# mspaintenjoyer/DepthEstimation

Hardware: AMD Instinct MI355X
Metric: disparity Mpix/s at 1080p d_max=128; 1/2/4/8-GPU scaling + %HBM roofline (higher is better)
Workload: dtype u8

## Files before the change

### depthestimation_amd/csrc/dsx_bm.hip

```cpp
#include "dsx_internal.h"
#include "dsx_partition.h"
#include "dsx_subpix.h"

constexpr int kWpe = 3;
constexpr int kWpeSsd = 4;

#ifndef DSX_ROWSTEP_PAIRTAIL
#define DSX_ROWSTEP_PAIRTAIL 0
#endif
#ifndef DSX_ROWSTEP_DIVQ
#define DSX_ROWSTEP_DIVQ 1
#endif
#ifndef DSX_ROWSTEP_OVERLAP
#define DSX_ROWSTEP_OVERLAP 1
#endif
#ifndef DSX_ROWSTEP_AHEAD
#define DSX_ROWSTEP_AHEAD 1
#endif
#ifndef DSX_ROWSTEP_SREF
#define DSX_ROWSTEP_SREF 0
#endif
#ifndef DSX_ROWSTEP_SARGS
#define DSX_ROWSTEP_SARGS DSX_ROWSTEP_SREF
#endif
constexpr bool kRowstepSref = DSX_ROWSTEP_SREF;
constexpr bool kRowstepSargs = DSX_ROWSTEP_SARGS;
constexpr bool kRowstepOverlap = DSX_ROWSTEP_OVERLAP;
constexpr bool kRowstepAhead = DSX_ROWSTEP_AHEAD;
constexpr bool kRowstepPairtail = DSX_ROWSTEP_PAIRTAIL;
constexpr bool kRowstepDivq = DSX_ROWSTEP_DIVQ;
#ifndef DSX_ROWSTEP_ATID
#define DSX_ROWSTEP_ATID 1
#endif
#ifndef DSX_ROWSTEP_KEY2
#define DSX_ROWSTEP_KEY2 1
#endif
#ifndef DSX_ROWSTEP_MERGE
#define DSX_ROWSTEP_MERGE 1
#endif
constexpr bool kRowstepMerge = DSX_ROWSTEP_MERGE;
constexpr bool kRowstepAtid = DSX_ROWSTEP_ATID;
constexpr bool kRowstepKey2 = DSX_ROWSTEP_KEY2;
#ifndef DSX_SEGSTART_AHEAD
#define DSX_SEGSTART_AHEAD 1
#endif
#ifndef DSX_SEGSTART_BATCH
#define DSX_SEGSTART_BATCH 1
#endif
#ifndef DSX_SEGSTART_SPART
#define DSX_SEGSTART_SPART 0
#endif
constexpr bool kSegstartAhead = DSX_SEGSTART_AHEAD;
constexpr bool kSegstartBatch = DSX_SEGSTART_BATCH;
constexpr bool kSegstartSpart = DSX_SEGSTART_SPART;

#include <algorithm>
#include <cstdio>
#include <cstdlib>
#include <cstring>
#include <mutex>
#include <type_traits>
#include <utility>
#include <vector>

namespace dsx {

typedef unsigned short u16x2 __attribute__((ext_vector_type(2)));
typedef uint32_t u32x2 __attribute__((ext_vector_type(2)));
__device__ __forceinline__ u32x2 lds_read_b64(const uint8_t *p) {
    return *(const volatile __attribute__((address_space(3))) u32x2 *)p;
}

__device__ __forceinline__ u16x2 as2(uint32_t v) { return __builtin_bit_cast(u16x2, v); }
__device__ __forceinline__ uint32_t as1(u16x2 v) { return __builtin_bit_cast(uint32_t, v); }
__device__ __forceinline__ int clampi2(int v, int lo, int hi) { return v < lo ? lo : (v > hi ? hi : v); }
__device__ __forceinline__ uint32_t umin2(uint32_t a, uint32_t b) { return a < b ? a : b; }
__device__ __forceinline__ u16x2 add_sub2(u16x2 a, u16x2 p, u16x2 q) { return as2(as1(a) + as1(p) - as1(q)); }
__device__ __forceinline__ int mad_i24(int a, int b, int c) {
    int r;
    asm("v_mad_i32_i24 %0, %1, %2, %3" : "=v"(r) : "v"(a), "v"(b), "v"(c));
    return r;
}
__device__ __forceinline__ uint32_t sad_hi_u8(uint32_t a, uint32_t b, uint32_t c) {
    return __builtin_amdgcn_sad_hi_u8(a, b, c);
}
__device__ __forceinline__ uint32_t min_shr1(uint32_t src, uint32_t key) {
    asm("s_nop 1\n\tv_min_u32_dpp %0, %1, %0 wave_shr:1 row_mask:0xf bank_mask:0xf" : "+v"(key) : "v"(src));
    return key;
}
#pragma clang diagnostic push
#pragma clang diagnostic ignored "-Winline-asm"
template <int OFF0, int STRIDE>
__device__ __forceinline__ void lds_store8_addtid(uint32_t m0base, const uint32_t (&v)[8]) {
    static_assert(OFF0 >= 0 && OFF0 + 7 * STRIDE < 65536, "16-bit offset field");
    asm volatile("s_mov_b32 m0, %8\n\ts_nop 0\n\t"
                 "ds_write_addtid_b32 %0 offset:%9\n\t"
                 "ds_write_addtid_b32 %1 offset:%10\n\t"
                 "ds_write_addtid_b32 %2 offset:%11\n\t"
                 "ds_write_addtid_b32 %3 offset:%12\n\t"
                 "ds_write_addtid_b32 %4 offset:%13\n\t"
                 "ds_write_addtid_b32 %5 offset:%14\n\t"
                 "ds_write_addtid_b32 %6 offset:%15\n\t"
                 "ds_write_addtid_b32 %7 offset:%16"
                 :
// ... 100 lines not shown
#endif
) {
    using G = Geo<R, SSD, NW>;
    constexpr int TX = G::TX, NC = G::NC, Dp = G::Dp, NT = G::NT, TPP = G::TPP, DSL = G::DSL, CB = G::CB,
                  PITCH = G::PITCH, NJ = G::NJ, SLOT = G::SLOT, NB = G::NB, NJ4 = (NJ + 3) / 4;
    constexpr int side = SIDE;
    const Bm2Args a = kargs_row<SIDE == 3>(a_in);
    constexpr bool FSS = SSD && !ABS && R <= 5 && (SIDE == 0 || SIDE == 3 || SIDE == 4);
    constexpr bool SGK = SIDE == 4;
    constexpr uint32_t OFF = FSS ? 0x4B000000u : 0u;
    constexpr int CW = (!FSS && (SSD || SIDE == 3)) ? 4 : 8, NCH = (NC + CW - 1) / CW;
    typedef typename std::conditional<FSS, float, typename std::conditional<SSD, uint32_t, u16x2>::type>::type acc_t;
    uint8_t *tile = smem + 4 * SLOT;

    constexpr bool LANE_RB = SSD && !ABS && NW >= 4;
    int ln = 0;
    if constexpr (LANE_RB)
        asm volatile("v_mbcnt_lo_u32_b32 %0, -1, 0\n\tv_mbcnt_hi_u32_b32 %0, -1, %0" : "=v"(ln));
    else
        ln = (int)threadIdx.x & 63;
    const int tid = LANE_RB ? (wvu << 6) + ln : (int)threadIdx.x;
    const int wv = LANE_RB ? wvu : tid >> 6;
    const int H = a.H, W = a.W, m = a.m, D = a.D;
    const int64_t stride = a.stride;
    const int d0 = SSD ? (wv * 64 + ln) : (wv * 128 + 2 * ln);
    const uint32_t padv = a.padv;
    const int PB = side == 1 ? (x0 - R + m) : (x0 - R - m + NC - 1);
    const int sgn = side == 1 ? 1 : -1;

    constexpr int NC4 = (NC + 3) / 4;
    constexpr bool RL2 = !SSD;
    uint32_t ofs_r = (uint32_t)(x0 - R + 4 * min(tid, NC4 - 1));
    uint32_t ofs_s = side == 1 ? (uint32_t)(PB + 4 * min(tid, NJ4 - 1)) : (uint32_t)(PB - 4 * min(tid, NJ4 - 1) - 3);
    constexpr bool MRG = kRowstepMerge && RL2 && FAST && SIDE != 3 && SIDE != 2 && !(SIDE == 4 && R >= 7);
    static_assert(!MRG || NJ4 + NC4 <= NT, "merged staging: a lane per staged dword");
    const bool m_s = tid < NJ4;
    const int m_r = min(tid - NJ4, NC4 - 1);
    const uint8_t *m_base = m_s ? a.src + fin + ofs_s : a.ref + fin + (uint32_t)(x0 - R + 4 * m_r);
    const bool m_dn = m_s && side != 1;
    const uint32_t m_sel0 = m_dn ? 0x0C0C0C03u : 0x0C0C0C00u, m_sel1 = m_dn ? 0x0C0C0C02u : 0x0C0C0C01u,
                   m_sel2 = m_dn ? 0x0C0C0C01u : 0x0C0C0C02u, m_sel3 = m_dn ? 0x0C0C0C00u : 0x0C0C0C03u;
    const uint32_t m_lane = m_s ? (uint32_t)(16 * tid) : (uint32_t)(G::SROW + 16 * m_r);
    auto ldm = [&](int r, uint32_t &w) __attribute__((always_inline)) {
        const int yy = clampi2(r, 0, H - 1);
        long ro = (long)yy * stride;
        asm("" : "+s"(ro));
        w = *reinterpret_cast<const uint32_t *>(m_base + ro);
    };
    auto stm = [&](uint8_t *sp, uint32_t w) __attribute__((always_inline)) {
        if (tid < NJ4 + NC4)
            *reinterpret_cast<uint4 *>(sp) = make_uint4(__builtin_amdgcn_perm(0u, w, m_sel0), __builtin_amdgcn_perm(0u, w, m_sel1),
                                                        __builtin_amdgcn_perm(0u, w, m_sel2), __builtin_amdgcn_perm(0u, w, m_sel3));
    };
    auto ld = [&](int r, uint32_t &w0, uint32_t &w1, uint32_t &w2, uint32_t &w3, uint32_t &rf) __attribute__((always_inline)) {
        const int yy = clampi2(r, 0, H - 1);
        const uint8_t *srow_ = a.src + fin + (long)yy * stride;
        const uint8_t *rrow_ = a.ref + fin + (long)yy * stride;
        if constexpr (RL2) {
            asm("" : "+s"(srow_));
            asm("" : "+s"(rrow_));
        }
        typedef typename std::conditional<RL2, gu8, const uint8_t>::type row8;
        typedef typename std::conditional<RL2, gu32, const uint32_t>::type row32;
        typedef typename std::conditional<RL2, uint32_t, int>::type rix;
        row8 *srow = (row8 *)srow_, *rrow = (row8 *)rrow_;
        const int tr = min(tid, NC4 - 1);
        if constexpr (FAST) {
            if constexpr (RL2) {
                rf = *reinterpret_cast<row32 *>(rrow + ofs_r);
            } else {
                rf = *reinterpret_cast<row32 *>(rrow + x0 - R + 4 * tr);
            }
        } else {
            uint32_t v = 0;
#pragma unroll
            for (int q = 0; q < 4; ++q) v |= (uint32_t)rrow[(rix)clampi2(x0 - R + 4 * tr + q, 0, W - 1)] << (8 * q);
            rf = v;
        }
        if constexpr (FAST) {
            const int tj = min(tid, NJ4 - 1);
            row8 *p;
            if constexpr (RL2) {
                p = srow + ofs_s;
            } else {
                p = side == 1 ? srow + PB + 4 * tj : (SIDE == 3 && NW == 1) ? srow + (PB - 4 * tj - 3) : srow + PB - 4 * tj - 3;
            }
            w0 = *reinterpret_cast<row32 *>(p);
            if constexpr (RL2) w1 = w2 = w3 = 0;
        } else {
            uint32_t v[4];
            int t4 = 4 * tid;
            if constexpr (!SSD && NW == 1 && SIDE == 3)
                asm volatile("" : "+v"(t4));
#pragma unroll
            for (int q = 0; q < 4; ++q) {
                const int j = min(t4 + q, NJ - 1);
                const int pp = PB + sgn * j;
                uint32_t t = srow[(rix)clampi2(pp, 0, W - 1)];
                if constexpr (FSS) t = __float_as_uint((float)t);
                v[q] = t;
            }
            w0 = v[0];
            w1 = v[1];
            w2 = v[2];
            w3 = v[3];
        }
// ... 140 lines not shown
                } else {
                    w[r] = 0;
                    e[r] = 0;
                    rf[r] = 0;
                }
            }
        };
        auto itrg = [&](int g, const uint32_t(&w)[4], const uint32_t(&e)[4], const uint32_t(&rf)[4]) __attribute__((always_inline)) {
            uint32_t P[5];
#pragma unroll
            for (int q = 0; q < 4; ++q) {
                const uint32_t b = 3 - q;
                const uint32_t lo = __builtin_amdgcn_perm(w[1], w[0], 0x0C0C0000u | ((4u + b) << 8) | b);
                const uint32_t hi = __builtin_amdgcn_perm(w[3], w[2], 0x0C0C0000u | ((4u + b) << 8) | b);
                P[q] = __builtin_amdgcn_perm(hi, lo, 0x05040100u);
            }
            {
                const uint32_t lo = __builtin_amdgcn_perm(e[1], e[0], 0x0C0C0400u);
                const uint32_t hi = __builtin_amdgcn_perm(e[3], e[2], 0x0C0C0400u);
                P[4] = __builtin_amdgcn_perm(hi, lo, 0x05040100u);
            }
            if (tid < NJ4) {
                uint4 *tp = reinterpret_cast<uint4 *>(smem + g * TPG + 32 * tid);
                tp[0] = make_uint4(P[0], P[1], P[1], P[2]);
                tp[1] = make_uint4(P[2], P[3], P[3], P[4]);
            }
            if (tid < NC4) {
                uint32_t Rv[4];
#pragma unroll
                for (int k = 0; k < 4; ++k) {
                    const uint32_t lo = __builtin_amdgcn_perm(rf[1], rf[0], 0x0C0C0000u | ((4u + k) << 8) | (uint32_t)k);
                    const uint32_t hi = __builtin_amdgcn_perm(rf[3], rf[2], 0x0C0C0000u | ((4u + k) << 8) | (uint32_t)k);
                    Rv[k] = __builtin_amdgcn_perm(hi, lo, 0x05040100u);
                }
                *reinterpret_cast<uint4 *>(smem + NGR * TPG + g * RG + 16 * tid) = make_uint4(Rv[0], Rv[1], Rv[2], Rv[3]);
            }
        };
        if constexpr (IBT) {
            uint32_t w[NGR][4], e[NGR][4], rf[NGR][4];
#pragma unroll
            for (int g = 0; g < NGR; ++g) ildg(g, w[g], e[g], rf[g]);
            __builtin_amdgcn_sched_barrier(0);
#pragma unroll
            for (int g = 0; g < NGR; ++g) itrg(g, w[g], e[g], rf[g]);
        } else {
#pragma unroll 1
            for (int g = 0; g < NGR; ++g) {
                uint32_t w[4], e[4], rf[4];
                ildg(g, w, e, rf);
                itrg(g, w, e, rf);
            }
        }
        block_sync<NW>();
        const uint8_t *tb = smem + d0 * 8;
        {
        uint32_t ae[NC], ao[NC];
#pragma unroll
        for (int c = 0; c < NC; ++c) ae[c] = ao[c] = 0;
        constexpr bool IAH = kSegstartAhead && R <= 5;
        if constexpr (IAH) {
#pragma unroll 1
            for (int g = 0; g < NGR; ++g) {
                uint32_t rv[2][4], p0[2][4], p1[2][4];
                auto ird = [&](auto qc) __attribute__((always_inline)) {
                    constexpr int q = decltype(qc)::value, c0 = 4 * q, t = q & 1;
                    const uint4 rr = *reinterpret_cast<const uint4 *>(smem + NGR * TPG + g * RG + 4 * c0);
                    rv[t][0] = rr.x; rv[t][1] = rr.y; rv[t][2] = rr.z; rv[t][3] = rr.w;
#pragma unroll
                    for (int c = 0; c < 4; ++c) {
                        if (c0 + c < NC) {
                            if constexpr (ABS) {
                                p0[t][c] = *reinterpret_cast<const uint32_t *>(tb + g * TPG + (NC - 1 - c0 - c) * 8);
                            } else {
                                const uint2 pr = *reinterpret_cast<const uint2 *>(tb + g * TPG + (NC - 1 - c0 - c) * 8);
                                p0[t][c] = pr.x;
                                p1[t][c] = pr.y;
                            }
                        }
                    }
                };
                auto isad = [&](auto qc) __attribute__((always_inline)) {
                    constexpr int q = decltype(qc)::value, c0 = 4 * q, t = q & 1;
#pragma unroll
                    for (int c = 0; c < 4; ++c) {
                        if (c0 + c < NC) {
                            ae[c0 + c] = __builtin_amdgcn_sad_u8(rv[t][c], p0[t][c], ae[c0 + c]);
                            if constexpr (!ABS) ao[c0 + c] = __builtin_amdgcn_sad_u8(rv[t][c], p1[t][c], ao[c0 + c]);
                        }
                    }
                };
                auto ichunk = [&](auto qc) __attribute__((always_inline)) {
                    constexpr int q = decltype(qc)::value;
                    if constexpr (q < NC4) {
                        __builtin_amdgcn_sched_barrier(0);
                        if constexpr (q + 1 < NC4) ird(std::integral_constant<int, q + 1>{});
                        __builtin_amdgcn_sched_barrier(0);
                        isad(qc);
                    }
                };
                ird(std::integral_constant<int, 0>{});
                ichunk(std::integral_constant<int, 0>{}); ichunk(std::integral_constant<int, 1>{});
                ichunk(std::integral_constant<int, 2>{}); ichunk(std::integral_constant<int, 3>{});
                ichunk(std::integral_constant<int, 4>{}); ichunk(std::integral_constant<int, 5>{});
                ichunk(std::integral_constant<int, 6>{}); ichunk(std::integral_constant<int, 7>{});
                ichunk(std::integral_constant<int, 8>{}); ichunk(std::integral_constant<int, 9>{});
                ichunk(std::integral_constant<int, 10>{}); ichunk(std::integral_constant<int, 11>{});
// ... 47 lines not shown
        }
    }
    block_sync<NW>();
#pragma unroll 1
    for (int i = 0; i <= 2 * R; ++i) {
        uint32_t nx = 0;
#pragma unroll
        for (int q = 0; q < NCH; ++q) {
            const int c0 = CW * q;
            uint32_t sw[CW + 1], rw[CW];
            float rf8[8];
            s_chunk(i, c0, sw, nx);
            if constexpr (FSS) ref_chunkf(i, c0, rf8);
            else ref_chunk(i, c0, rw);
#pragma unroll
            for (int c = 0; c < CW; ++c) {
                if (c0 + c < NC) {
                    if constexpr (FSS) {
                        const float t = rf8[c] - __uint_as_float(sw[c]);
                        cs[c0 + c] = __builtin_fmaf(t, t, cs[c0 + c]);
                    } else if constexpr (ABS) {
                        cs[c0 + c] = __builtin_amdgcn_sad_u16(rw[c], sw[c], cs[c0 + c]);
                    } else if constexpr (SSD) {
                        const int t = (int)rw[c] - (int)sw[c];
                        cs[c0 + c] += (uint32_t)__mul24(t, t);
                    } else {
                        cs[c0 + c] = as2(sad_hi_u8(rw[c], pair_e1(sw, c), __builtin_amdgcn_sad_u8(rw[c], pair_e0(sw, c), as1(cs[c0 + c]))));
                    }
                }
            }
            if constexpr (SSD) __builtin_amdgcn_sched_barrier(0);
        }
    }
    }
    block_sync<NW>();

    for (int q = tid; q < TX * (Dp - D); q += NT) {
        const int k = q / (Dp - D), d = D + (q - k * (Dp - D));
        if constexpr (SSD) *reinterpret_cast<uint32_t *>(tile + k * PITCH + d * 4) = padv + OFF;
        else *reinterpret_cast<uint16_t *>(tile + k * PITCH + d * 2) = (uint16_t)padv;
    }
    block_sync<NW>();

    const bool edge = side == 1 && (x0 + m < 0 || x0 + TX - 1 + m + Dp - 1 > W - 1);
    const bool dodd = !SSD && (D & 1);
    const bool lane_writes = d0 < D;

    uint32_t stg = (MRG ? m_lane : (uint32_t)(16 * tid)) + (uint32_t)((2 - (yb & 1) * 2) * SLOT);
    constexpr bool PTAIL = kRowstepPairtail && !SSD && SIDE == 0 && NW == 1;
    constexpr bool DIVQ = kRowstepDivq && !SSD && SIDE == 0;
    uint32_t kp0 = 0, kp1 = 0;
    constexpr bool CUQ = !SSD && SIDE == 0 && NW == 1 && R < 6 && kRowstepKey2 && !PTAIL;
    constexpr bool OVL = kRowstepOverlap && CUQ, AHD = kRowstepAhead && CUQ;
    constexpr int CQ = 4, NQ = (NC + CQ - 1) / CQ;
    constexpr bool SREF = kRowstepSref && CUQ && FAST && OVL && R < 5;
    constexpr bool SRA = kRowstepSargs && CUQ && OVL && R < 5;
    static_assert(!SREF || NQ == NC4, "one reference dword per column chunk");
    uint32_t qn[NC4 + 1] = {}, qo[NC4 + 1] = {}, shn = 0, sho = 0;
    auto sld = [&](int r, uint32_t(&q)[NC4 + 1], uint32_t &sh) __attribute__((always_inline)) {
        const int yy = clampi2(r, 0, H - 1);
        const uintptr_t p = (uintptr_t)(a.ref + fin + (long)yy * stride + (x0 - R));
        typedef const __attribute__((address_space(4))) uint8_t cu8;
        cu8 *b = (cu8 *)(p & ~(uintptr_t)3);
#pragma unroll
        for (int i = 0; i < NC4; ++i) q[i] = *(cu32 *)(b + 4 * i);
        q[NC4] = *(cu32 *)(b + ((((uint32_t)p + 4u * NC4 - 1u) & ~3u) - ((uint32_t)p & ~3u)));
        sh = ((uint32_t)p & 3u) * 8u;
    };
    auto sbyte = [](uint32_t w, int c) __attribute__((always_inline)) -> uint32_t {
        return c == 3 ? w >> 24 : (w >> (8 * c)) & 0xFFu;
    };
    constexpr int RPS = NQ >= 10 ? 1 : 2, NRS = 8 / RPS;
    static_assert(NQ >= NRS + 2, "a column chunk per stage up to the element keys");
    const int ek = tid / TPP, eh = tid % TPP, ex = x0 + ek;
    const uint8_t *epx = tile + ek * PITCH + eh * DSL * CB;
    uint4 etv[2] = {};
    uint32_t ekmin = 0, ecb = 0, egblk = 0, ecm = 0, ecp = 0;
    int eb = 0, ef = 0, eden = 1;
    bool esp = false;
    auto emin8 = [](uint4 v) __attribute__((always_inline)) -> uint32_t {
        const u16x2 mm = __builtin_elementwise_min(__builtin_elementwise_min(as2(v.x), as2(v.y)),
                                                   __builtin_elementwise_min(as2(v.z), as2(v.w)));
        return umin2(mm.x, mm.y);
    };
    auto estage = [&](auto sc, int ey, auto rl, const Bm2Args &er) __attribute__((always_inline)) {
        constexpr int s = decltype(sc)::value;
        constexpr bool RL = decltype(rl)::value;
        auto pick = [&]() __attribute__((always_inline)) -> const Bm2Args & {
            if constexpr (RL) return er;
            else return a;
        };
        const Bm2Args &ea = pick();
        static_assert(!OVL || (NB == 8 && TPP == 2), "overlapped epilogue: 64 disparities per lane, two lanes per pixel");
        constexpr int GB = Dp / 8 <= 16 ? 4 : (Dp / 8 <= 32 ? 5 : 6);
        if constexpr (s <= NRS) {
            if constexpr (s == 0) ekmin = 0xFFFFFFFFu;
#pragma unroll
            for (int j = 0; j < (s > 0 ? RPS : 0); ++j) ekmin = umin2(ekmin, (emin8(etv[j]) << GB) | (uint32_t)(RPS * (s - 1) + j));
            if constexpr (s < NRS) {
#pragma unroll
                for (int j = 0; j < RPS; ++j) etv[j] = *reinterpret_cast<const uint4 *>(epx + 16 * (RPS * s + j));
            } else {
                const uint32_t kmin = gmin<TPP>(ekmin | (uint32_t)(eh * 8));
                ecb = kmin >> GB;
                egblk = kmin & ((1u << GB) - 1u);
                etv[0] = *reinterpret_cast<const uint4 *>(epx + 16 * (egblk & 7u));
            }
        } else if constexpr (s == NRS + 1) {
            const uint32_t w4[4] = {etv[0].x, etv[0].y, etv[0].z, etv[0].w};
            uint32_t k8 = 0xFFFFFFFFu;
#pragma unroll
            for (int q = 0; q < 4; ++q) {
                k8 = umin2(k8, (w4[q] << 16) | (uint32_t)(2 * q));
                k8 = umin2(k8, (w4[q] & 0xFFFF0000u) | (uint32_t)(2 * q + 1));
            }
            const uint32_t dl = (int)(egblk / 8) == eh ? egblk * 8 + (k8 & 7u) : 0xFFFFu;
            eb = (int)gmin<TPP>(dl);
            const uint16_t *pc = reinterpret_cast<const uint16_t *>(tile + ek * PITCH) + eb;
            ecm = pc[-1];
            ecp = pc[1];
        } else if constexpr (s == NRS + 2) {
            esp = ea.subpix && eb > 0 && eb < D - 1;
            int32_t den = (int32_t)ecm + (int32_t)ecp - 2 * (int32_t)ecb;
            eden = den < 1 ? 1 : den;
            const int32_t num = ((int32_t)ecm - (int32_t)ecp) * 16 + eden;
            const int32_t q = DIVQ ? subpix_quot(num, 2 * eden) : div_trunc_small(num, 2 * eden);
            ef = eb * 16 + (esp ? q : 0);
        } else {
            const uint32_t padv_e = RL ? er.padv : padv;
            bool valid = ex < W && ex >= m + D - 1 && ex <= W - 1 + m;
            if (ea.uniq > 0) {
                const int rel = eb - eh * DSL;
                uint32_t nm = 0xFFFFFFFFu;
#pragma unroll
                for (int i = 0; i < 8; ++i) {
                    const bool hit = rel >= 8 * i - 1 && rel <= 8 * i + 8;
                    nm = hit ? nm : umin2(nm, emin8(*reinterpret_cast<const uint4 *>(epx + 16 * i)));
                }
                const int ib0 = (rel - 1) >> 3, ib1 = (rel + 1) >> 3;
#pragma unroll
                for (int t = 0; t < 2; ++t) {
                    const int ib = t == 0 ? ib0 : ib1;
                    if (ib >= 0 && ib < 8 && (t == 0 || ib1 != ib0)) {
                        const uint4 v = *reinterpret_cast<const uint4 *>(epx + 16 * ib);
                        const uint32_t c8[8] = {v.x & 0xFFFFu, v.x >> 16, v.y & 0xFFFFu, v.y >> 16,
                                                v.z & 0xFFFFu, v.z >> 16, v.w & 0xFFFFu, v.w >> 16};
#pragma unroll
                        for (int e = 0; e < 8; ++e) {
                            const int dd = 8 * ib + e - rel;
                            nm = (dd > 1 || dd < -1) ? umin2(nm, c8[e]) : nm;
                        }
                    }
                }
                nm = gmin<TPP>(nm);
                const uint32_t real_max = padv_e < (1u << 24) ? padv_e : (1u << 24);
                if (nm < real_max && nm * (uint32_t)(100 - ea.uniq) < ecb * 100u) valid = false;
            }
            if (eh == 0 && ex < W) {
                const long o = fout + (long)ey * W + ex;
                const int16_t fx = valid ? (int16_t)(m * 16 + ef) : (int16_t)((m - 1) * 16);
                if (ea.out_fixed) ea.out_fixed[o] = fx;
                if (ea.out_float) {
                    if (ea.float_mode == 0) {
                        ea.out_float[o] = (float)fx * 0.0625f;
                    } else {
                        float pf = (float)(m + eb);
                        if (esp) pf = (float)(m + eb) + (float)((int32_t)ecm - (int32_t)ecp) / (float)(2 * eden);
                        ea.out_float[o] = valid ? pf : (float)(m - 1);
                    }
                }
            }
        }
    };
    if constexpr (SREF) {
        sld(yb + 1 + R, qn, shn);
        sld(yb - R, qo, sho);
    }
    for (int y = yb; y < ye; ++y) {
        const Bm2Args &a = kargs_row<SIDE == 3>(a_in);
#ifdef DSX_STAMPS
        ++nsteps;
#endif
        DSX_STAMP(0);
        if (a.prio) {
            const int dn = done0 + (y - yb);
            const int q = RL2 ? (int)(((uint32_t)(pe[0] - 1 - dn) >> 31) + ((uint32_t)(pe[1] - 1 - dn) >> 31) +
                                      ((uint32_t)(pe[2] - 1 - dn) >> 31))
                              : (dn >= pe[0]) + (dn >= pe[1]) + (dn >= pe[2]);
            if (q != qcur) {
                qcur = q;
                switch (q) {
                    case 0: __builtin_amdgcn_s_setprio(3); break;
                    case 1: __builtin_amdgcn_s_setprio(2); break;
                    case 2: __builtin_amdgcn_s_setprio(1); break;
                    default: __builtin_amdgcn_s_setprio(0); break;
                }
            }
        }
        if constexpr (RL2 && FAST && !MRG) asm volatile("" : "+v"(ofs_r), "+v"(ofs_s));
        const int par = (y & 1) * 2;
        const bool more = y + 1 < ye;
        uint32_t pn0 = 0, pn1 = 0, pn2 = 0, pn3 = 0, pnr = 0, po0 = 0, po1 = 0, po2 = 0, po3 = 0, por = 0;
        if constexpr (MRG) {
            ldm(y + 1 + R, pn0);
            ldm(y - R, po0);
        } else if (RL2 || more) {
            ld(y + 1 + R, pn0, pn1, pn2, pn3, pnr);
            ld(y - R, po0, po1, po2, po3, por);
        }
        if constexpr (FSS) {
          if (y > yb) {
#pragma unroll
            for (int q = 0; q < (NC + 3) / 4; ++q) {
                const int c0 = 4 * q;
                const uint4 rn = *reinterpret_cast<const uint4 *>(smem + par * SLOT + G::SROW + 4 * c0);
                const uint4 ro = *reinterpret_cast<const uint4 *>(smem + (par + 1) * SLOT + G::SROW + 4 * c0);
                const float rn4[4] = {__uint_as_float(rn.x), __uint_as_float(rn.y), __uint_as_float(rn.z), __uint_as_float(rn.w)};
                const float ro4[4] = {__uint_as_float(ro.x), __uint_as_float(ro.y), __uint_as_float(ro.z), __uint_as_float(ro.w)};
                const uint8_t *bn = smem + par * SLOT + d0 * 4, *bo = smem + (par + 1) * SLOT + d0 * 4;
#pragma unroll
                for (int c = 0; c < 4; ++c) {
                    if (c0 + c < NC) {
                        const float sn = *reinterpret_cast<const float *>(bn + (NC - 1 - c0 - c) * 4);
                        const float so = *reinterpret_cast<const float *>(bo + (NC - 1 - c0 - c) * 4);
                        const float tn = rn4[c] - sn, to = ro4[c] - so;
                        cs[c0 + c] = __builtin_fmaf(-to, to, __builtin_fmaf(tn, tn, cs[c0 + c]));
                    }
                }
            }
          }
        } else if constexpr (OVL || AHD) {
          if (y > yb) {
            uint32_t sn[2][CQ + 1], so[2][CQ + 1], rn[2][CQ], ro[2][CQ];
            uint32_t nxn = 0, nxo = 0;
            auto rd = [&](auto qc) __attribute__((always_inline)) {
                constexpr int q = decltype(qc)::value, c0 = CQ * q, t = AHD ? (q & 1) : 0;
                const uint8_t *bn = (const uint8_t *)__builtin_assume_aligned(smem + par * SLOT + d0 * 4, 8);
                const uint8_t *bo = (const uint8_t *)__builtin_assume_aligned(smem + (par + 1) * SLOT + d0 * 4, 8);
                if constexpr (!SREF) {
                    const uint4 vn = *reinterpret_cast<const uint4 *>(smem + par * SLOT + G::SROW + 4 * c0);
                    const uint4 vo = *reinterpret_cast<const uint4 *>(smem + (par + 1) * SLOT + G::SROW + 4 * c0);
                    rn[t][0] = vn.x; rn[t][1] = vn.y; rn[t][2] = vn.z; rn[t][3] = vn.w;
                    ro[t][0] = vo.x; ro[t][1] = vo.y; ro[t][2] = vo.z; ro[t][3] = vo.w;
                }
                sn[t][0] = c0 == 0 ? *reinterpret_cast<const uint32_t *>(bn + NC * 4) : nxn;
                so[t][0] = c0 == 0 ? *reinterpret_cast<const uint32_t *>(bo + NC * 4) : nxo;
#pragma unroll
                for (int c = 1; c < CQ; c += 2) {
                    if (c0 + c < NC) {
                        const u32x2 pn = lds_read_b64(bn + (NC - 1 - c0 - c) * 4);
                        const u32x2 po = lds_read_b64(bo + (NC - 1 - c0 - c) * 4);
                        sn[t][c + 1] = pn.x; sn[t][c] = pn.y; nxn = pn.x;
                        so[t][c + 1] = po.x; so[t][c] = po.y; nxo = po.x;
                    }
                }
            };
            auto sads = [&](auto qc) __attribute__((always_inline)) {
                constexpr int q = decltype(qc)::value, c0 = CQ * q, t = AHD ? (q & 1) : 0;
                uint32_t wn = 0, wo = 0;
                if constexpr (SREF) {
                    uint32_t hn = qn[q + 1], ho = qo[q + 1];
                    asm("" : "+s"(hn));
                    asm("" : "+s"(ho));
                    wn = (uint32_t)((((uint64_t)hn << 32) | qn[q]) >> shn);
                    wo = (uint32_t)((((uint64_t)ho << 32) | qo[q]) >> sho);
                }
#pragma unroll
                for (int c = 0; c < CQ; ++c) {
                    if (c0 + c < NC) {
                        const uint32_t bn = SREF ? sbyte(wn, c) : rn[t][c], bo = SREF ? sbyte(wo, c) : ro[t][c];
                        const uint32_t en = sad_hi_u8(bn, sn[t][c], __builtin_amdgcn_sad_u8(bn, sn[t][c + 1], as1(cs[c0 + c])));
                        const uint32_t lo = sad_hi_u8(bo, so[t][c], __builtin_amdgcn_sad_u8(bo, so[t][c + 1], 0u));
                        uint32_t v = en - lo;
                        if constexpr (OVL) asm volatile("" : "+v"(v));
                        cs[c0 + c] = as2(v);
                    }
                }
            };
            auto chunk = [&](auto qc) __attribute__((always_inline)) {
                constexpr int q = decltype(qc)::value;
                if constexpr (q < NQ) {
                    __builtin_amdgcn_sched_barrier(0);
                    if constexpr (OVL && q < NRS + 3) estage(qc, y - 1, std::false_type{}, a);
                    if constexpr (!AHD) rd(qc);
                    else if constexpr (q + 1 < NQ) rd(std::integral_constant<int, q + 1>{});
                    __builtin_amdgcn_sched_barrier(0);
                    sads(qc);
                }
            };
            if constexpr (AHD) rd(std::integral_constant<int, 0>{});
            chunk(std::integral_constant<int, 0>{}); chunk(std::integral_constant<int, 1>{});
            chunk(std::integral_constant<int, 2>{}); chunk(std::integral_constant<int, 3>{});
            chunk(std::integral_constant<int, 4>{}); chunk(std::integral_constant<int, 5>{});
            chunk(std::integral_constant<int, 6>{}); chunk(std::integral_constant<int, 7>{});
            chunk(std::integral_constant<int, 8>{}); chunk(std::integral_constant<int, 9>{});
            chunk(std::integral_constant<int, 10>{}); chunk(std::integral_constant<int, 11>{});
            static_assert(NQ <= 12 && NQ >= 7, "chunks of the overlapped column update");
            __builtin_amdgcn_sched_barrier(0);
            if constexpr (SREF) {
                sld(y + 1 + R, qn, shn);
                sld(y - R, qo, sho);
            }
            const Bm2Args &ea = kargs_row<SRA>(a);
            if constexpr (SRA) __builtin_amdgcn_sched_barrier(0);
            if constexpr (OVL) {
                if constexpr (NQ < NRS + 3) estage(std::integral_constant<int, NRS + 2>{}, y - 1, std::integral_constant<bool, SRA>{}, ea);
                estage(std::integral_constant<int, NRS + 3>{}, y - 1, std::integral_constant<bool, SRA>{}, ea);
            }
          }
        } else if (y > yb) {
            uint32_t nxn = 0, nxo = 0;
#pragma unroll
            for (int q = 0; q < NCH; ++q) {
                const int c0 = CW * q;
                uint32_t sn[CW + 1], so[CW + 1], rn[CW], ro[CW];
                ref_chunk(par, c0, rn);
                ref_chunk(par + 1, c0, ro);
                s_chunk(par, c0, sn, nxn);
                s_chunk(par + 1, c0, so, nxo);
#pragma unroll
                for (int c = 0; c < CW; ++c) {
                    if (c0 + c < NC) {
                        if constexpr (ABS) {
                            cs[c0 + c] = __builtin_amdgcn_sad_u16(rn[c], sn[c], cs[c0 + c]) -
                                         __builtin_amdgcn_sad_u16(ro[c], so[c], 0u);
                        } else if constexpr (SSD) {
                            const int tn = (int)rn[c] - (int)sn[c];
                            const int to = (int)ro[c] - (int)so[c];
                            const int nto = (int)so[c] - (int)ro[c];
                            cs[c0 + c] = (uint32_t)mad_i24(to, nto, mad_i24(tn, tn, (int)cs[c0 + c]));
                        } else {
                            const uint32_t en = sad_hi_u8(rn[c], pair_e1(sn, c), __builtin_amdgcn_sad_u8(rn[c], pair_e0(sn, c), as1(cs[c0 + c])));
                            const uint32_t lo = sad_hi_u8(ro[c], pair_e1(so, c), __builtin_amdgcn_sad_u8(ro[c], pair_e0(so, c), 0u));
                            cs[c0 + c] = as2(en - lo);
                        }
                    }
                }
            }
        }
        DSX_STAMP(1);
        DSX_STAMP(2);
        {
            uint8_t *tb = tile + d0 * CB;
            constexpr bool ATID = kRowstepAtid && !SSD && SIDE != 3;
            auto abits = [](acc_t v) __attribute__((always_inline)) -> uint32_t {
                if constexpr (FSS) return __float_as_uint(v);
                else if constexpr (SSD) return v;
                else return as1(v);
            };
            acc_t acc = cs[0];
            if constexpr (FSS) acc = 8388608.0f + cs[0];
#pragma unroll
            for (int c = 1; c <= 2 * R; ++c) {
                if constexpr (SSD) acc += cs[c];
                else acc = as2(as1(acc) + as1(cs[c]));
            }
            if constexpr (side == 3) {
                static_assert(SSD || NW <= 4, "SAD exit slots: 16 B of padding per tile row");
                const int ks = a.kshift;
                const uint32_t selE = d0 < D ? 0x05040100u : 0x0D0D0D0Du;
// ... 80 lines not shown
                }
            } else if (ATID && lane_writes) {
                static_assert(!ATID || (TX % 8 == 0 && G::LDW * CB == 256), "addtid: a lane's tile bytes are 4 * lane");
                if constexpr (ATID) {
                const uint32_t mb = lds_offset(tile) + (uint32_t)wvu * (uint32_t)(G::LDW * CB);
                auto grp = [&](auto k0c) __attribute__((always_inline)) {
                    constexpr int k0 = decltype(k0c)::value;
                    uint32_t v[8];
#pragma unroll
                    for (int j = 0; j < 8; ++j) {
                        if (k0 + j > 0) acc = add_sub2(acc, cs[k0 + j + 2 * R], cs[k0 + j - 1]);
                        v[j] = as1(acc);
                    }
                    lds_store8_addtid<k0 * PITCH, PITCH>(mb, v);
                };
                grp(std::integral_constant<int, 0>{});
                grp(std::integral_constant<int, 8>{});
                grp(std::integral_constant<int, 16>{});
                grp(std::integral_constant<int, 24>{});
                }
            } else if (lane_writes) {
#pragma unroll
                for (int k = 0; k < TX; ++k) {
                    if (k > 0) {
                        if constexpr (FSS) acc = (acc - cs[k - 1]) + cs[k + 2 * R];
                        else if constexpr (SSD) acc = acc + cs[k + 2 * R] - cs[k - 1];
                        else acc = add_sub2(acc, cs[k + 2 * R], cs[k - 1]);
                    }
                    if constexpr (SSD) *reinterpret_cast<uint32_t *>(tb + k * PITCH) = abits(acc);
                    else *reinterpret_cast<uint32_t *>(tb + k * PITCH) = as1(acc);
                }
            }
            if (dodd && d0 + 1 == D) {
                for (int k = 0; k < TX; ++k) *reinterpret_cast<uint16_t *>(tb + k * PITCH + 2) = (uint16_t)padv;
            }
            if (edge && lane_writes) {
                const int base = x0 + m + d0;
                for (int k = 0; k < TX; ++k) {
                    const int p0 = base + k;
                    if constexpr (SSD) {
                        if (p0 < 0 || p0 > W - 1) *reinterpret_cast<uint32_t *>(tb + k * PITCH) = padv;
                    } else {
                        if (p0 < 0 || p0 > W - 1) *reinterpret_cast<uint16_t *>(tb + k * PITCH) = (uint16_t)padv;
                        if (p0 + 1 < 0 || p0 + 1 > W - 1) *reinterpret_cast<uint16_t *>(tb + k * PITCH + 2) = (uint16_t)padv;
                    }
                }
            }
        }
        DSX_STAMP(3);
        if constexpr (kRowstepAtid && !SSD && SIDE != 3 && NW > 1) lds_drain();
        block_sync<NW>();
        DSX_STAMP(4);
        if constexpr (RL2) {
            if constexpr (MRG) {
                if (more) {
                    stm(smem + stg, pn0);
                    stm(smem + stg + SLOT, po0);
                }
                stg = (2 * m_lane + (uint32_t)(2 * SLOT)) - stg;
            } else if constexpr (SIDE != 3) {
                if (more) {
                    st_at(smem + stg, pn0, pn1, pn2, pn3, pnr);
                    st_at(smem + stg + SLOT, po0, po1, po2, po3, por);
                }
                stg = (uint32_t)(32 * tid + 2 * SLOT) - stg;
            } else if (more) {
                st(par ^ 2, pn0, pn1, pn2, pn3, pnr);
                st((par ^ 2) + 1, po0, po1, po2, po3, por);
            }
        }
        DSX_STAMP(5);
        if constexpr (side == 2) {
            constexpr int CPP = Dp * CB / 16;
            for (int q = tid; q < TX * CPP; q += NT) {
                const int k = q / CPP, off = (q - k * CPP) * 16;
                const int x = x0 + k;
                if (x < W) {
                    const uint4 v = *reinterpret_cast<const uint4 *>(tile + k * PITCH + off);
                    *reinterpret_cast<uint4 *>(reinterpret_cast<uint8_t *>(a.vol) + ((size_t)fout + (size_t)y * W + x) * (Dp * CB) + off) = v;
                }
            }
        } else if constexpr (!OVL) {
            const int k = tid / TPP, h = tid % TPP;
            const int x = x0 + k;
            const uint8_t *px = tile + k * PITCH + h * DSL * CB;
            uint32_t bs[NB];
#pragma unroll
            for (int i = 0; i < NB; ++i) {
                if constexpr (SSD) {
                    const uint4 v0 = *reinterpret_cast<const uint4 *>(px + 32 * i);
                    const uint4 v1 = *reinterpret_cast<const uint4 *>(px + 32 * i + 16);
                    bs[i] = umin2(umin2(umin2(v0.x, v0.y), umin2(v0.z, v0.w)), umin2(umin2(v1.x, v1.y), umin2(v1.z, v1.w))) - OFF;
                } else {
                    const uint4 v = *reinterpret_cast<const uint4 *>(px + 16 * i);
                    const u16x2 mm = __builtin_elementwise_min(__builtin_elementwise_min(as2(v.x), as2(v.y)),
                                                               __builtin_elementwise_min(as2(v.z), as2(v.w)));
                    bs[i] = umin2(mm.x, mm.y);
                }
            }
            constexpr bool KEYS = SIDE == 3 || R >= 6;
            constexpr bool KEY2 = kRowstepKey2 && !KEYS && !SSD;
            uint32_t cb, dl;
            if constexpr (KEYS) {
                constexpr int GB = Dp / 8 <= 16 ? 4 : (Dp / 8 <= 32 ? 5 : 6);
                uint32_t kmin = 0xFFFFFFFFu;
    #pragma unroll
                for (int i = 0; i < NB; ++i) kmin = umin2(kmin, (bs[i] << GB) | (uint32_t)(h * NB + i));
                kmin = gmin<TPP>(kmin);
                cb = kmin >> GB;
                const int gblk = (int)(kmin & ((1u << GB) - 1u));
                dl = 0xFFFFu;
                if (gblk / NB == h) {
                    const int bsel = gblk - h * NB;
                    uint32_t k8 = 0xFFFFFFFFu;
                    if constexpr (SSD) {
                        const uint4 v0 = *reinterpret_cast<const uint4 *>(px + 32 * bsel);
                        const uint4 v1 = *reinterpret_cast<const uint4 *>(px + 32 * bsel + 16);
                        const uint32_t c8[8] = {v0.x - OFF, v0.y - OFF, v0.z - OFF, v0.w - OFF,
                                                v1.x - OFF, v1.y - OFF, v1.z - OFF, v1.w - OFF};
    #pragma unroll
                        for (int q = 0; q < 8; ++q) k8 = umin2(k8, (c8[q] << 3) | (uint32_t)q);
                    } else {
// ... 134 lines not shown
                                float *rowp = a.out_float + ro;
                                asm("" : "+s"(rowp));
                                *(gf32 *)((gw8 *)rowp + 4u * xh) = a.float_mode == 0 ? (float)fx * 0.0625f : (tvalid ? pf : (float)(m - 1));
                            }
                        }
                    } else {
                        kp0 = c0;
                        kp1 = c1;
                    }
                } else {
                int32_t f = b * 16;
                float pf = (float)(m + b);
                if (a.subpix && b > 0 && b < D - 1) {
                    int32_t cm, cp;
                    const uint8_t *pk = tile + k * PITCH;
                    if constexpr (SSD) {
                        cm = (int32_t)(reinterpret_cast<const uint32_t *>(pk)[b - 1] - OFF);
                        cp = (int32_t)(reinterpret_cast<const uint32_t *>(pk)[b + 1] - OFF);
                    } else {
                        cm = reinterpret_cast<const uint16_t *>(pk)[b - 1];
                        cp = reinterpret_cast<const uint16_t *>(pk)[b + 1];
                    }
                    int32_t den = cm + cp - 2 * (int32_t)cb;
                    den = den < 1 ? 1 : den;
                    if constexpr (DIVQ) f += subpix_quot((cm - cp) * 16 + den, 2 * den);
                    else f += div_trunc_small((cm - cp) * 16 + den, 2 * den);
                    if (a.float_mode == 1) pf = (float)(m + b) + (float)(cm - cp) / (float)(2 * den);
                }
                if (h == 0 && x < W) {
                    if (lr_on) a.dstar[o] = valid ? (int16_t)b : (int16_t)-1;
                    const int16_t fx = valid ? (int16_t)(m * 16 + f) : (int16_t)((m - 1) * 16);
                    if constexpr (SGK) {
                        a.dstar[o] = fx;
                        if (valid)
                            atomicMin(a.sg_keys + fout + (long)y * W + (x - m - b),
                                      (cb << a.kshift) | (((1u << a.kshift) - 1u) - (uint32_t)b));
                    }
                    if (a.out_fixed) a.out_fixed[o] = fx;
                    if (a.out_float) a.out_float[o] = a.float_mode == 0 ? (float)fx * 0.0625f : (valid ? pf : (float)(m - 1));
                }
                }
            }
        }
        if (!RL2 && more) {
            st(par ^ 2, pn0, pn1, pn2, pn3, pnr);
            st((par ^ 2) + 1, po0, po1, po2, po3, por);
        }
        DSX_STAMP(6);
        block_sync<NW>();
        DSX_STAMP(7);
    }
    if constexpr (OVL) {
        auto dr = [&](auto sc) __attribute__((always_inline)) {
            if constexpr (decltype(sc)::value <= NRS + 3) estage(sc, ye - 1, std::false_type{}, a);
        };
        dr(std::integral_constant<int, 0>{}); dr(std::integral_constant<int, 1>{}); dr(std::integral_constant<int, 2>{});
        dr(std::integral_constant<int, 3>{}); dr(std::integral_constant<int, 4>{}); dr(std::integral_constant<int, 5>{});
        dr(std::integral_constant<int, 6>{}); dr(std::integral_constant<int, 7>{}); dr(std::integral_constant<int, 8>{});
        dr(std::integral_constant<int, 9>{}); dr(std::integral_constant<int, 10>{}); dr(std::integral_constant<int, 11>{});
    }
}

template <int R, bool SSD, int NW, int SIDE, bool ABS>
__global__ __launch_bounds__(64 * NW) __attribute__((amdgpu_waves_per_eu((SSD && NW >= 4) ? kWpeSsd : kWpe))) void bm2(Bm2Args a) {
    using G = Geo<R, SSD, NW>;
    constexpr int TX = G::TX, NT = G::NT, NC = G::NC, NJ = G::NJ;
    constexpr int side = SIDE;
    extern __shared__ __attribute__((aligned(16))) uint8_t smem[];
    const int tid = threadIdx.x;
    const int wvu = __builtin_amdgcn_readfirstlane(tid >> 6);
    const int H = a.H, W = a.W, m = a.m;
    if (a.timeline && wvu == 0 && __lane_id() == 0) a.timeline[4 * blockIdx.x] = __builtin_amdgcn_s_memrealtime();
#ifdef DSX_STAMPS
    uint64_t ph[8] = {0, 0, 0, 0, 0, 0, 0, 0};
    uint64_t t_prev = 0;
    uint64_t nsteps = 0;
#endif
    constexpr bool SPART = kSegstartSpart && R <= 5;
    int sp0 = 0, sp1 = 0;
    if constexpr (SPART) {
        typedef const __attribute__((address_space(4))) int ci32;
        ci32 *pp = (ci32 *)((uintptr_t)a.part + 4 * (uintptr_t)blockIdx.x);
        sp0 = pp[0];
        sp1 = pp[1];
    }

    if ((side == 0 || side == 3 || side == 4) && (a.out_fixed || a.out_float)) {
        const int xa = a.strip_begin * TX, xb = min(W, (a.strip_begin + a.strip_count) * TX);
        const int nin = xa + (W - xb);
        const int total = nin * H * a.nframes;
        const int16_t fi = (int16_t)((m - 1) * 16);
        for (int q = blockIdx.x * NT + tid; q < total; q += gridDim.x * NT) {
            const int y = q / nin;
            const int c = q - y * nin;
            const int x = c < xa ? c : xb + (c - xa);
            const long o = (long)y * W + x;
            if (a.out_fixed) a.out_fixed[o] = fi;
            if (a.out_float) a.out_float[o] = (float)(m - 1);
            if constexpr (side == 4) a.dstar[o] = fi;
        }
    }

    if ((side == 3 || side == 4) && a.lr_reset_n > 0) {
        uint32_t *kr = a.lr_reset;
        const int64_t n = a.lr_reset_n, stride = (int64_t)gridDim.x * NT;
        const int64_t t0 = (int64_t)blockIdx.x * NT + tid;
        if (((uintptr_t)kr & 15u) == 0) {
// ... 98 lines not shown
    }
    const std::vector<int> part = bm2_partition(k.NG, k.S, k.sb, k.nframes, k.H, k.XL, k.XU, TX, k.w8, k.nlev, k.w);
    int *d = nullptr;
    hipError_t e = hipMalloc(&d, part.size() * sizeof(int));
    if (e != hipSuccess) return e;
    e = hipMemcpy(d, part.data(), part.size() * sizeof(int), hipMemcpyHostToDevice);
    if (e != hipSuccess) {
        (void)hipFree(d);
        return e;
    }
    cache.emplace_back(k, d);
    *out = d;
    return hipSuccess;
}

template <int R, bool SSD, int NW, int SIDE, bool ABS = false>
static hipError_t launch_bm2_side(const Bm2Args &a, hipStream_t st) {
    using G = Geo<R, SSD, NW>;
    constexpr int SM = G::SMEM + ((SIDE == 3 && !SSD) ? G::XRB * NW : 0);
    const void *fn = (const void *)bm2<R, SSD, NW, SIDE, ABS>;
    static int blocks_per_cu[64] = {};
    static int num_cu[64] = {};
    int dev = 0;
    hipError_t e = hipGetDevice(&dev);
    if (e != hipSuccess) return e;
    if (dev < 0 || dev >= 64) return hipErrorInvalidDevice;
    std::lock_guard<std::mutex> lock(launch_mutex());
    if (!blocks_per_cu[dev]) {
        e = hipFuncSetAttribute(fn, hipFuncAttributeMaxDynamicSharedMemorySize, SM);
        if (e != hipSuccess) return e;
        int nb = 0;
        e = hipOccupancyMaxActiveBlocksPerMultiprocessor(&nb, fn, G::NT, SM);
        if (e != hipSuccess) return e;
        int cus = 0;
        e = hipDeviceGetAttribute(&cus, hipDeviceAttributeMultiprocessorCount, dev);
        if (e != hipSuccess) return e;
        const char *adj = getenv("DSX_BLOCKS_PER_CU_ADJ");
        const int nbr = nb + (adj ? atoi(adj) : 0);
        blocks_per_cu[dev] = nbr > 1 ? nbr : 1;
        num_cu[dev] = cus > 0 ? cus : 1;
    }
    const long T = (long)a.strip_count * a.nframes * a.H;
    long grid = (long)blocks_per_cu[dev] * num_cu[dev];
    static const bool small_grid = [] {
        const char *e = getenv("DSX_SMALL_GRID");
        return !(e && *e == '0');
    }();
    if (small_grid && !ABS && T < grid * (2L * R + 1) && blocks_per_cu[dev] >= 3) grid = (long)num_cu[dev] * (blocks_per_cu[dev] * 2 / 3);
    static const bool flight_grid = [] {
        const char *e = getenv("DSX_FLIGHT_GRID");
        return !(e && *e == '0');
    }();
    if (flight_grid && a.in_flight && NW == 1 && blocks_per_cu[dev] >= 3) {
        const long g23 = (long)num_cu[dev] * (blocks_per_cu[dev] * 2 / 3);
        if (g23 < grid) grid = g23;
    }
    if (a.grid_override > 0) grid = a.grid_override;
    if (grid > T) grid = T;
    if (grid < 1) grid = 1;
    static const bool verbose = getenv("DSX_VERBOSE") != nullptr;
    if (verbose)
        fprintf(stderr, "[dsx] bm2<R=%d,SSD=%d,NW=%d,SIDE=%d> grid %ld (%d/CU) smem %d\n", R, (int)SSD, NW, SIDE, grid,
                blocks_per_cu[dev], SM);
    Bm2Args la = a;
    la.nlev = 1;
    if (grid == (long)blocks_per_cu[dev] * num_cu[dev] && a.nframes == 1) {
        const int lv = blocks_per_cu[dev] * NW / 4;
        la.nlev = lv < 1 ? 1 : (lv > 4 ? 4 : lv);
    }
    {
        constexpr int NJ4 = (G::NJ + 3) / 4, NC4 = (G::NC + 3) / 4, NC = G::NC;
        const int W = a.W, m = a.m;
        PartKey k;
        memset(&k, 0, sizeof(k));
        k.dev = dev, k.NG = (int)grid, k.S = a.strip_count, k.sb = a.strip_begin, k.nframes = a.nframes, k.H = a.H;
        if (SIDE == 1) {
            k.XL = std::max(R - m, R);
            k.XU = std::min(W - 1 - 4 * NJ4 + R - m, W - 1 + R - 4 * NC4 + 1);
        } else {
            k.XL = std::max(4 * NJ4 + R + m - NC + 1, R);
            k.XU = std::min(W - 1 + R + m - NC + 1, W - 1 + R - 4 * NC4 + 1);
        }
        k.w8 = a.slow_w8, k.nlev = la.nlev;
        for (int i = 0; i < 4; ++i) k.w[i] = la.nlev > 1 ? a.agew[i] : 64;
        e = bm2_partition_dev(k, G::TX, &la.part);
        if (e != hipSuccess) return e;
    }
    hipLaunchKernelGGL((bm2<R, SSD, NW, SIDE, ABS>), dim3((unsigned)grid), dim3(G::NT), SM, st, la);
    return hipGetLastError();
}

template <int R, bool SSD, int NW>
static hipError_t launch_bm2_one(const Bm2Args &a, hipStream_t st) {
    switch (a.side) {
        case 0: return a.sg_keys ? launch_bm2_side<R, SSD, NW, 4>(a, st) : launch_bm2_side<R, SSD, NW, 0>(a, st);
        case 1: return launch_bm2_side<R, SSD, NW, 1>(a, st);
        case 3: return launch_bm2_side<R, SSD, NW, 3>(a, st);
        default: return launch_bm2_side<R, SSD, NW, 2>(a, st);
    }
}

template <int R>
static hipError_t launch_bm2_sad1(const Bm2Args &a, hipStream_t st) {
    switch (a.side) {
        case 0: return a.sg_keys ? launch_bm2_side<R, true, 1, 4, true>(a, st) : launch_bm2_side<R, true, 1, 0, true>(a, st);
        case 1: return launch_bm2_side<R, true, 1, 1, true>(a, st);
        case 3: return launch_bm2_side<R, true, 1, 3, true>(a, st);
// ... 52 lines not shown
```

Before: 47330.

## Defer epilogue disparity stores past row sync and shrink in-flight grid

Adds a default-on STORELATE mode that computes the final epilogue stage's fixed/float disparity into registers and writes it to global memory after the row's block sync, moving the store latency off the overlapped column-update path. Also adds off-by-default options to stage next-row LDS stores earlier and to hoist the first step's row loads behind the batched init loads. For the in-flight grid path with SAD side 0, the grid drops from 2/3 to 1/2 of blocks per CU. Deferring the store costs extra live registers, and the smaller grid trades occupancy for less contention.

```diff
diff --git a/depthestimation_amd/csrc/dsx_bm.hip b/depthestimation_amd/csrc/dsx_bm.hip
--- a/depthestimation_amd/csrc/dsx_bm.hip
+++ b/depthestimation_amd/csrc/dsx_bm.hip
@@ -23,6 +23,14 @@
 #ifndef DSX_ROWSTEP_SARGS
 #define DSX_ROWSTEP_SARGS DSX_ROWSTEP_SREF
 #endif
+#ifndef DSX_ROWSTEP_STAGEAHEAD
+#define DSX_ROWSTEP_STAGEAHEAD 0
+#endif
+constexpr bool kRowstepStageahead = DSX_ROWSTEP_STAGEAHEAD;
+#ifndef DSX_ROWSTEP_STORELATE
+#define DSX_ROWSTEP_STORELATE 1
+#endif
+constexpr bool kRowstepStorelate = DSX_ROWSTEP_STORELATE;
 constexpr bool kRowstepSref = DSX_ROWSTEP_SREF;
 constexpr bool kRowstepSargs = DSX_ROWSTEP_SARGS;
 constexpr bool kRowstepOverlap = DSX_ROWSTEP_OVERLAP;
@@ -50,6 +58,10 @@
 #ifndef DSX_SEGSTART_SPART
 #define DSX_SEGSTART_SPART 0
 #endif
+#ifndef DSX_SEGSTART_ROW0
+#define DSX_SEGSTART_ROW0 0
+#endif
+constexpr bool kSegstartRow0 = DSX_SEGSTART_ROW0;
 constexpr bool kSegstartAhead = DSX_SEGSTART_AHEAD;
 constexpr bool kSegstartBatch = DSX_SEGSTART_BATCH;
 constexpr bool kSegstartSpart = DSX_SEGSTART_SPART;
@@ -256,6 +268,8 @@
             *reinterpret_cast<uint4 *>(sp) = make_uint4(__builtin_amdgcn_perm(0u, w, m_sel0), __builtin_amdgcn_perm(0u, w, m_sel1),
                                                         __builtin_amdgcn_perm(0u, w, m_sel2), __builtin_amdgcn_perm(0u, w, m_sel3));
     };
+    constexpr bool SR0 = kSegstartRow0 && kSegstartBatch && MRG && R <= 4 && (SIDE == 0 || SIDE == 4);
+    uint32_t sr_n = 0, sr_o = 0;
     auto ld = [&](int r, uint32_t &w0, uint32_t &w1, uint32_t &w2, uint32_t &w3, uint32_t &rf) __attribute__((always_inline)) {
         const int yy = clampi2(r, 0, H - 1);
         const uint8_t *srow_ = a.src + fin + (long)yy * stride;
@@ -502,6 +516,12 @@
             }
         }
         block_sync<NW>();
+        if constexpr (SR0) {
+            static_assert(!SR0 || IBT, "the first step's rows ride behind the batched init loads");
+            ldm(yb + 1 + R, sr_n);
+            ldm(yb - R, sr_o);
+            __builtin_amdgcn_sched_barrier(0);
+        }
         const uint8_t *tb = smem + d0 * 8;
         {
         uint32_t ae[NC], ao[NC];
@@ -655,6 +675,10 @@
     uint32_t kp0 = 0, kp1 = 0;
     constexpr bool CUQ = !SSD && SIDE == 0 && NW == 1 && R < 6 && kRowstepKey2 && !PTAIL;
     constexpr bool OVL = kRowstepOverlap && CUQ, AHD = kRowstepAhead && CUQ;
+    constexpr bool STA = kRowstepStageahead && OVL;
+    constexpr bool STL = kRowstepStorelate && OVL;
+    int e_fx = 0;
+    float e_pf = 0.0f;
     constexpr int CQ = 4, NQ = (NC + CQ - 1) / CQ;
     constexpr bool SREF = kRowstepSref && CUQ && FAST && OVL && R < 5;
     constexpr bool SRA = kRowstepSargs && CUQ && OVL && R < 5;
@@ -686,9 +710,17 @@
                                                    __builtin_elementwise_min(as2(v.z), as2(v.w)));
         return umin2(mm.x, mm.y);
     };
-    auto estage = [&](auto sc, int ey, auto rl, const Bm2Args &er) __attribute__((always_inline)) {
+    auto estore = [&](int ey, const Bm2Args &ea) __attribute__((always_inline)) {
+        if (eh == 0 && ex < W) {
+            const long o = fout + (long)ey * W + ex;
+            if (ea.out_fixed) ea.out_fixed[o] = (int16_t)e_fx;
+            if (ea.out_float) ea.out_float[o] = ea.float_mode == 0 ? (float)(int16_t)e_fx * 0.0625f : e_pf;
+        }
+    };
+    auto estage = [&](auto sc, int ey, auto rl, const Bm2Args &er, auto dfr) __attribute__((always_inline)) {
         constexpr int s = decltype(sc)::value;
         constexpr bool RL = decltype(rl)::value;
+        constexpr bool DFR = decltype(dfr)::value;
         auto pick = [&]() __attribute__((always_inline)) -> const Bm2Args & {
             if constexpr (RL) return er;
             else return a;
@@ -759,7 +791,14 @@
                 const uint32_t real_max = padv_e < (1u << 24) ? padv_e : (1u << 24);
                 if (nm < real_max && nm * (uint32_t)(100 - ea.uniq) < ecb * 100u) valid = false;
             }
-            if (eh == 0 && ex < W) {
+            if constexpr (DFR) {
+                e_fx = valid ? (int16_t)(m * 16 + ef) : (int16_t)((m - 1) * 16);
+                if (eh == 0 && ex < W && ea.out_float && ea.float_mode != 0) {
+                    float pf = (float)(m + eb);
+                    if (esp) pf = (float)(m + eb) + (float)((int32_t)ecm - (int32_t)ecp) / (float)(2 * eden);
+                    e_pf = valid ? pf : (float)(m - 1);
+                }
+            } else if (eh == 0 && ex < W) {
                 const long o = fout + (long)ey * W + ex;
                 const int16_t fx = valid ? (int16_t)(m * 16 + ef) : (int16_t)((m - 1) * 16);
                 if (ea.out_fixed) ea.out_fixed[o] = fx;
@@ -778,6 +817,13 @@
     if constexpr (SREF) {
         sld(yb + 1 + R, qn, shn);
         sld(yb - R, qo, sho);
+    }
+    if constexpr (SR0) {
+        if (yb + 1 < ye) {
+            stm(smem + stg, sr_n);
+            stm(smem + stg + SLOT, sr_o);
+        }
+        stg = (2 * m_lane + (uint32_t)(2 * SLOT)) - stg;
     }
     for (int y = yb; y < ye; ++y) {
         const Bm2Args &a = kargs_row<SIDE == 3>(a_in);
@@ -804,7 +850,12 @@
         const int par = (y & 1) * 2;
         const bool more = y + 1 < ye;
         uint32_t pn0 = 0, pn1 = 0, pn2 = 0, pn3 = 0, pnr = 0, po0 = 0, po1 = 0, po2 = 0, po3 = 0, por = 0;
-        if constexpr (MRG) {
+        if constexpr (SR0) {
+            if (y > yb) {
+                ldm(y + 1 + R, pn0);
+                ldm(y - R, po0);
+            }
+        } else if constexpr (MRG) {
             ldm(y + 1 + R, pn0);
             ldm(y - R, po0);
         } else if (RL2 || more) {
@@ -884,7 +935,7 @@
                 constexpr int q = decltype(qc)::value;
                 if constexpr (q < NQ) {
                     __builtin_amdgcn_sched_barrier(0);
-                    if constexpr (OVL && q < NRS + 3) estage(qc, y - 1, std::false_type{}, a);
+                    if constexpr (OVL && q < NRS + 3) estage(qc, y - 1, std::false_type{}, a, std::false_type{});
                     if constexpr (!AHD) rd(qc);
                     else if constexpr (q + 1 < NQ) rd(std::integral_constant<int, q + 1>{});
                     __builtin_amdgcn_sched_barrier(0);
@@ -900,6 +951,22 @@
             chunk(std::integral_constant<int, 10>{}); chunk(std::integral_constant<int, 11>{});
             static_assert(NQ <= 12 && NQ >= 7, "chunks of the overlapped column update");
             __builtin_amdgcn_sched_barrier(0);
+            if constexpr (STA) {
+                if constexpr (MRG) {
+                    if (more) {
+                        stm(smem + stg, pn0);
+                        stm(smem + stg + SLOT, po0);
+                    }
+                    stg = (2 * m_lane + (uint32_t)(2 * SLOT)) - stg;
+                } else {
+                    if (more) {
+                        st_at(smem + stg, pn0, pn1, pn2, pn3, pnr);
+                        st_at(smem + stg + SLOT, po0, po1, po2, po3, por);
+                    }
+                    stg = (uint32_t)(32 * tid + 2 * SLOT) - stg;
+                }
+                __builtin_amdgcn_sched_barrier(0);
+            }
             if constexpr (SREF) {
                 sld(y + 1 + R, qn, shn);
                 sld(y - R, qo, sho);
@@ -907,8 +974,8 @@
             const Bm2Args &ea = kargs_row<SRA>(a);
             if constexpr (SRA) __builtin_amdgcn_sched_barrier(0);
             if constexpr (OVL) {
-                if constexpr (NQ < NRS + 3) estage(std::integral_constant<int, NRS + 2>{}, y - 1, std::integral_constant<bool, SRA>{}, ea);
-                estage(std::integral_constant<int, NRS + 3>{}, y - 1, std::integral_constant<bool, SRA>{}, ea);
+                if constexpr (NQ < NRS + 3) estage(std::integral_constant<int, NRS + 2>{}, y - 1, std::integral_constant<bool, SRA>{}, ea, std::false_type{});
+                estage(std::integral_constant<int, NRS + 3>{}, y - 1, std::integral_constant<bool, SRA>{}, ea, std::integral_constant<bool, STL>{});
             }
           }
         } else if (y > yb) {
@@ -1095,22 +1162,26 @@
         block_sync<NW>();
         DSX_STAMP(4);
         if constexpr (RL2) {
+            [[maybe_unused]] const bool late = STA ? (!SR0 && y == yb) : (!SR0 || y > yb);
             if constexpr (MRG) {
-                if (more) {
+                if (more && late) {
                     stm(smem + stg, pn0);
                     stm(smem + stg + SLOT, po0);
                 }
-                stg = (2 * m_lane + (uint32_t)(2 * SLOT)) - stg;
+                if (late) stg = (2 * m_lane + (uint32_t)(2 * SLOT)) - stg;
             } else if constexpr (SIDE != 3) {
-                if (more) {
+                if (more && late) {
                     st_at(smem + stg, pn0, pn1, pn2, pn3, pnr);
                     st_at(smem + stg + SLOT, po0, po1, po2, po3, por);
                 }
-                stg = (uint32_t)(32 * tid + 2 * SLOT) - stg;
+                if (late) stg = (uint32_t)(32 * tid + 2 * SLOT) - stg;
             } else if (more) {
                 st(par ^ 2, pn0, pn1, pn2, pn3, pnr);
                 st((par ^ 2) + 1, po0, po1, po2, po3, por);
             }
+        }
+        if constexpr (STL) {
+            if (y > yb) estore(y - 1, a);
         }
         DSX_STAMP(5);
         if constexpr (side == 2) {
@@ -1351,7 +1422,7 @@
     }
     if constexpr (OVL) {
         auto dr = [&](auto sc) __attribute__((always_inline)) {
-            if constexpr (decltype(sc)::value <= NRS + 3) estage(sc, ye - 1, std::false_type{}, a);
+            if constexpr (decltype(sc)::value <= NRS + 3) estage(sc, ye - 1, std::false_type{}, a, std::false_type{});
         };
         dr(std::integral_constant<int, 0>{}); dr(std::integral_constant<int, 1>{}); dr(std::integral_constant<int, 2>{});
         dr(std::integral_constant<int, 3>{}); dr(std::integral_constant<int, 4>{}); dr(std::integral_constant<int, 5>{});
@@ -1556,7 +1627,8 @@
         return !(e && *e == '0');
     }();
     if (flight_grid && a.in_flight && NW == 1 && blocks_per_cu[dev] >= 3) {
-        const long g23 = (long)num_cu[dev] * (blocks_per_cu[dev] * 2 / 3);
+        const bool half = !SSD && SIDE == 0;
+        const long g23 = (long)num_cu[dev] * (half ? blocks_per_cu[dev] / 2 : blocks_per_cu[dev] * 2 / 3);
         if (g23 < grid) grid = g23;
     }
     if (a.grid_override > 0) grid = a.grid_override;
```

Result: faster. 48100, median of 6 (+1.6%).
